# PolyChord/PolyChordLite

Measured on AMD Instinct MI355X. Metric: likelihood evals/sec, 20D Gaussian nlive=2000, higher is better.
Workload: dtype f64; 1 GPU; configs[1]: 20-D Gaussian, nlive=2000, num_repeats=40, one full run per step; batch_chains=1000, parallelism=repeat-sharded x1, mode=one run at a time per GPU; R runs in step: roofline.in_step

## Files before the change

### polychordlite_amd/csrc/pc_engine.hip

```cpp
#include "pc_state.h"
#include "pc_resume.h"
#include "pc_prior_table.h"
#include "pc_launch.h"
#include "pc_plan.h"
#include <cstdio>
#include <cstdlib>
#include <cstring>
#include <cstdarg>
#include <cmath>
#include <vector>
#include <memory>
#include <string>
#include <chrono>
#include <algorithm>
#include <map>
#include <unordered_map>
#include <atomic>
#include <mutex>
#include <thread>
#include <functional>
#include <exception>
#include <ucontext.h>
#include <array>
#include <sys/mman.h>
// ... 140 lines not shown
    {
        int dev = 0; (void)hipGetDevice(&dev);
        {
            std::lock_guard<std::mutex> g(m);
            for (size_t i = events.size(); i-- > 0;)
                if (events[i].first == dev) { hipEvent_t e = events[i].second; events.erase(events.begin() + i); return e; }
        }
        hipEvent_t e; HIPCHK(hipEventCreate(&e)); return e;
    }
    void put_event(hipEvent_t e) { int dev = 0; (void)hipGetDevice(&dev); std::lock_guard<std::mutex> g(m); events.push_back({dev, e}); }
    std::vector<std::pair<int, hipEvent_t>> sync_events;
    hipEvent_t get_sync_event()
    {
        int dev = 0; (void)hipGetDevice(&dev);
        {
            std::lock_guard<std::mutex> g(m);
            for (size_t i = sync_events.size(); i-- > 0;)
                if (sync_events[i].first == dev) { hipEvent_t e = sync_events[i].second; sync_events.erase(sync_events.begin() + i); return e; }
        }
        hipEvent_t e; HIPCHK(hipEventCreateWithFlags(&e, hipEventDisableTiming)); return e;
    }
    void put_sync_event(hipEvent_t e) { int dev = 0; (void)hipGetDevice(&dev); std::lock_guard<std::mutex> g(m); sync_events.push_back({dev, e}); }
};
HandlePool &hpool() { static HandlePool *p = new HandlePool; return *p; }

#define PC_COPY_N 96
#define PC_COPY_PIECE 4096u
struct PcCopyBatch { const void *src[PC_COPY_N]; void *dst[PC_COPY_N]; unsigned bytes[PC_COPY_N]; };
__global__ __launch_bounds__(256) void k_copy_batch(PcCopyBatch b)
{
    const int i = blockIdx.x;
    const unsigned n = b.bytes[i];
    const char *s = (const char *)b.src[i]; char *d = (char *)b.dst[i];
    if ((((uintptr_t)s | (uintptr_t)d) & 7u) == 0u) {
        const unsigned n8 = n >> 3;
        for (unsigned k = threadIdx.x; k < n8; k += 256) ((unsigned long long *)d)[k] = ((const unsigned long long *)s)[k];
        for (unsigned k = (n8 << 3) + threadIdx.x; k < n; k += 256) d[k] = s[k];
    } else for (unsigned k = threadIdx.x; k < n; k += 256) d[k] = s[k];
}
static void pc_copy_many(const std::vector<std::array<uintptr_t, 3>> &reqs, hipStream_t q)
{
    PcCopyBatch b; int n = 0;
    auto go = [&] { if (n) { hipLaunchKernelGGL(k_copy_batch, dim3(n), dim3(256), 0, q, b); n = 0; } };
    for (const auto &r : reqs) {
        size_t left = r[2]; uintptr_t d = r[0], s = r[1];
        while (left) {
            const unsigned c = (unsigned)std::min<size_t>(left, PC_COPY_PIECE);
            b.dst[n] = (void *)d; b.src[n] = (const void *)s; b.bytes[n] = c; ++n;
            d += c; s += c; left -= c;
            if (n == PC_COPY_N) go();
        }
    }
    go();
}

__global__ void k_engine_spin(long long ticks) { const long long t0 = wall_clock64(); while (wall_clock64() - t0 < ticks) {} }
static bool streams_overlap_test(hipStream_t a, hipStream_t b)
{
    auto both = [&] {
        (void)hipStreamSynchronize(a); (void)hipStreamSynchronize(b);
        const auto t0 = std::chrono::steady_clock::now();
        hipLaunchKernelGGL(k_engine_spin, dim3(1), dim3(64), 0, a, 10000LL);
        hipLaunchKernelGGL(k_engine_spin, dim3(1), dim3(64), 0, b, 10000LL);
        (void)hipStreamSynchronize(a); (void)hipStreamSynchronize(b);
        return std::chrono::duration<double>(std::chrono::steady_clock::now() - t0).count();
    };
    static std::atomic<bool> warmed{false};
    if (!warmed.exchange(true)) (void)both();
    const double two = std::min(both(), both());
    if (pc_env().debug == 5) std::fprintf(stderr, "polychord_hip dbg streams %p %p: both %.1f us\n", (void *)a, (void *)b, two * 1e6);
    return two < 170e-6;
}
struct StreamClasses {
    std::mutex mm;
    std::map<void *, int> cls;
    std::vector<hipStream_t> reps;
    int known(hipStream_t x) { std::lock_guard<std::mutex> g(mm); auto it = cls.find((void *)x); return it == cls.end() ? -1 : it->second; }
    int classify(hipStream_t x)
    {
        std::lock_guard<std::mutex> g(mm);
        auto it = cls.find((void *)x);
        if (it != cls.end()) return it->second;
        int c = -1;
        for (size_t r = 0; r < reps.size() && c < 0; ++r) if (!streams_overlap_test(reps[r], x)) c = (int)r;
        if (c < 0) { c = (int)reps.size(); reps.push_back(x); }
        cls[(void *)x] = c;
        return c;
    }
};
static StreamClasses &sclasses() { static StreamClasses *p = new StreamClasses; return *p; }
static hipStream_t stream_avoiding(std::vector<int> avoid, bool known_only = false);
static hipStream_t stream_beside(std::initializer_list<hipStream_t> others, bool known_only = false)
{
    if (pc_env().side_pick_off) return hpool().get_stream();
    std::vector<int> avoid;
    for (hipStream_t o : others) if (o) { const int c = known_only ? sclasses().known(o) : sclasses().classify(o); if (c >= 0) avoid.push_back(c); }
    return stream_avoiding(avoid, known_only);
}
static hipStream_t stream_avoiding(std::vector<int> avoid, bool known_only)
{
    auto fits = [&](int c) { return c >= 0 && std::find(avoid.begin(), avoid.end(), c) == avoid.end(); };
    if (hipStream_t k = hpool().take_stream_if([&](hipStream_t x) { return fits(sclasses().known(x)); })) return k;
    if (known_only) {
        if (hipStream_t k = hpool().take_stream_if([&](hipStream_t x) { return sclasses().known(x) >= 0; })) return k;
        return hpool().get_stream();
    }
// ... 1289 lines not shown
    {
        const int nprior = cfg.nprior <= 0 ? cfg.nlive : cfg.nprior, nT = S.nT;
        double *rows = dalloc<double>((size_t)nprior * nT), *rl = dalloc<double>(nprior);
        std::vector<double> keep_rows; keep_rows.reserve((size_t)nprior * nT);
        std::vector<double> hrows, hl(nprior);
        int have = 0, attempt0 = 0, last_attempt = -1;
        long long nlike = 0;
        bool direct = true;
        while (have < nprior) {
            pc_count(path, launch_traits());
            if (pc_launch_generate_live(&S, attempt0, nprior, rows, rl, st)) {
                if (pc_rtc_wanted(&S) && pc_rtc_error()) engine_fail(PC_RC_SETTINGS, "%.480s", pc_rtc_error());
                engine_fail(PC_RC_NDIMS, "nDims > 256 unsupported");
            }
            HIPCHK(hipMemcpyAsync(hl.data(), rl, sizeof(double) * nprior, hipMemcpyDeviceToHost, st));
            HIPCHK(hipStreamSynchronize(st));
            int nvalid = 0;
            for (int i = 0; i < nprior; ++i) nvalid += hl[i] > cfg.logzero;
            if (nvalid == nprior && have == 0) { have = nprior; nlike = nprior; last_attempt = nprior - 1; break; }
            direct = false;
            hrows.resize((size_t)nprior * nT);
            HIPCHK(hipMemcpy(hrows.data(), rows, sizeof(double) * (size_t)nprior * nT, hipMemcpyDeviceToHost));
            for (int i = 0; i < nprior && have < nprior; ++i)
                if (hl[i] > cfg.logzero) { keep_rows.insert(keep_rows.end(), hrows.begin() + (size_t)i * nT, hrows.begin() + (size_t)(i + 1) * nT); have++; nlike++; last_attempt = attempt0 + i; }
                else ndiscarded++;
            attempt0 += nprior;
        }
        if (!direct) HIPCHK(hipMemcpy(rows, keep_rows.data(), sizeof(double) * (size_t)nprior * nT, hipMemcpyHostToDevice));
        pc_launch_install_live(&S, rows, nprior, st);
        h_ctl->nlike = nlike; h_ctl->nlike_device = nlike;
        HIPCHK(hipMemcpyAsync(&S.ctl->nlike, &h_ctl->nlike, sizeof(long long), hipMemcpyHostToDevice, st));
        HIPCHK(hipStreamSynchronize(st));
        if (S.seq_mode) {
            int a = last_attempt + 1;
            for (; S.ngrade <= 1; ++a) {
                double l1 = 0.0;
                pc_count(path, launch_traits());
                (void)pc_launch_generate_live(&S, a, 1, rows, rl, st);
                HIPCHK(hipMemcpyAsync(&l1, rl, sizeof(double), hipMemcpyDeviceToHost, st));
                HIPCHK(hipStreamSynchronize(st));
                if (l1 > cfg.logzero) break;
            }
            h_ctl->seq = (unsigned long long)(a + (S.ngrade <= 1 ? 1 : 0)) * S.D;
            HIPCHK(hipMemcpy(&S.ctl->seq, &h_ctl->seq, sizeof(unsigned long long), hipMemcpyHostToDevice));
        }
        dfree(rows); dfree(rl);
        call_dumper(2);
        if (nprior > cfg.nlive) {
            pc_count(path, PcTrimLive{}); pc_launch_consume(&S, 2, 0, st);
            read_ctl();
        }
    }

    void stream_dead()
    {
        const size_t nd = (size_t)h_ctl->ndead;
        if (!h_dead || nd > h_dead_cap || nd <= h_dead_copied) return;
        if (ev_apply) HIPCHK(hipStreamWaitEvent(st_copy, ev_apply, 0));
        HIPCHK(hipMemcpyAsync(h_dead + h_dead_copied * S.nT, S.dead + h_dead_copied * S.nT,
                              sizeof(double) * (nd - h_dead_copied) * S.nT, hipMemcpyDeviceToHost, st_copy));
        h_dead_copied = nd;
    }

    void export_resume(PcResume &r)
    {
        HIPCHK(hipStreamSynchronize(st));
        const int D = S.D, nT = S.nT, nc = h_ctl->ncluster, ncd = std::min(h_ctl->ncluster_dead, S.maxc_dead), maxc = S.maxc;
        r = PcResume{};
        r.nDims = D; r.nDerived = S.nDer; r.ndead = h_ctl->ndead; r.ncluster = nc; r.ncluster_dead = ncd;
        {
            long ng[PC_MAX_GRADE];
            grade_counts(ng);
            r.grade_dims.clear(); r.num_repeats.clear(); r.nlike.clear();
            for (int g = 0; g < S.ngrade; ++g) {
                r.grade_dims.push_back((g + 1 < S.ngrade ? S.g_off[g + 1] : D) - S.g_off[g]);
                r.num_repeats.push_back(S.g_nr[g]); r.nlike.push_back(ng[g]);
            }
        }
        r.logZ = h_ctl->logZ; r.logZ2 = h_ctl->logZ2; r.logX_last_update = h_ctl->logX_last_update;
        r.thin_posterior = cfg.boost_posterior < 0.0 ? 1.0 : cfg.boost_posterior / (double)S.nr;
        auto take = [&](const double *p) { auto v = dl(p, std::max(1, nc)); v.resize(nc); return v; };
        r.logLp = take(S.logLp); r.logXp = take(S.logXp); r.logZXp = take(S.logZXp); r.logZp = take(S.logZp);
        r.logZp2 = take(S.logZp2); r.logZpXp = take(S.logZpXp);
        auto xq = dl(S.XpXq, (size_t)maxc * maxc);
        r.logXpXq.assign((size_t)nc * nc, 0.0);
        for (int q = 0; q < nc; ++q) for (int p = 0; p < nc; ++p) r.logXpXq[(size_t)q * nc + p] = xq[(size_t)p * maxc + q];
        r.logZp_dead = dl(S.logZp_dead, std::max(1, ncd)); r.logZp_dead.resize(ncd);
        r.logZp2_dead = dl(S.logZp2_dead, std::max(1, ncd)); r.logZp2_dead.resize(ncd);
        auto cov = dl(S.cov, (size_t)std::max(1, nc) * D * D), ch = dl(S.chol, (size_t)std::max(1, nc) * D * D);
        r.covmat.assign((size_t)nc * D * D, 0.0); r.cholesky.assign((size_t)nc * D * D, 0.0);
        for (int c = 0; c < nc; ++c) for (int j = 0; j < D; ++j) for (int a = 0; a < D; ++a) {
            r.covmat[((size_t)c * D + j) * D + a] = cov[((size_t)c * D + a) * D + j];
            r.cholesky[((size_t)c * D + j) * D + a] = ch[((size_t)c * D + a) * D + j];
        }
        auto cn = dl(S.cl_n, std::max(1, nc)); auto cl = dl(S.cl_list, (size_t)maxc * S.Ncap);
        auto rows = dl(S.live, (size_t)S.Ncap * nT); auto uid = dl(S.cl_uid, std::max(1, nc));
        r.nlive.assign(nc, 0); r.imin.assign(nc, 1); r.live.assign(nc, {}); r.nphantom.assign(nc, 0); r.phantom.assign(nc, {});
        for (int c = 0; c < nc; ++c) {
            r.nlive[c] = cn[c];
            double lo = PC_HUGE;
            for (int k = 0; k < cn[c]; ++k) {
                const double *row = rows.data() + (size_t)cl[(size_t)c * S.Ncap + k] * nT;
                r.live[c].insert(r.live[c].end(), row, row + nT);
                if (row[S.l0] < lo) { lo = row[S.l0]; r.imin[c] = k + 1; }
            }
        }
        const int nph = h_ctl->nphantom;
        auto ph = dl(S.phantom, (size_t)std::max(1, nph) * nT); auto pc = dl(S.ph_cuid, std::max(1, nph));
        for (int j = 0; j < nph; ++j)
            for (int c = 0; c < nc; ++c)
                if (uid[c] == pc[j]) { r.phantom[c].insert(r.phantom[c].end(), ph.begin() + (size_t)j * nT, ph.begin() + (size_t)(j + 1) * nT); r.nphantom[c]++; break; }
        r.dead = dl(S.dead, (size_t)std::max(1, r.ndead) * nT); r.dead.resize((size_t)r.ndead * nT);
        r.logweights = dl(S.dead_logw, std::max(1, r.ndead)); r.logweights.resize(r.ndead);
// ... 90 lines not shown
        put(S.logZp, r.logZp); put(S.logZXp, r.logZXp); put(S.logZp2, r.logZp2); put(S.logZpXp, r.logZpXp);
        { std::vector<double> t(maxc, 0.0); std::copy(r.logXp.begin(), r.logXp.end(), t.begin()); ul(S.logXp, t); }
        std::vector<double> xq((size_t)maxc * maxc, 0.0);
        for (int q = 0; q < nc; ++q) for (int p = 0; p < nc; ++p) xq[(size_t)p * maxc + q] = r.logXpXq[(size_t)q * nc + p];
        ul(S.XpXq, xq);
        std::vector<double> cov((size_t)maxc * D * D, 0.0), ch((size_t)maxc * D * D, 0.0);
        for (int c = 0; c < maxc; ++c) for (int a = 0; a < D; ++a) { cov[((size_t)c * D + a) * D + a] = 1.0; ch[((size_t)c * D + a) * D + a] = 1.0; }
        for (int c = 0; c < nc; ++c) for (int j = 0; j < D; ++j) for (int a = 0; a < D; ++a) {
            cov[((size_t)c * D + a) * D + j] = r.covmat[((size_t)c * D + j) * D + a];
            ch[((size_t)c * D + a) * D + j] = r.cholesky[((size_t)c * D + j) * D + a];
        }
        ul(S.cov, cov); ul(S.chol, ch);
        const int ncd = std::min(r.ncluster_dead, S.maxc_dead);
        { std::vector<double> a(r.logZp_dead.begin(), r.logZp_dead.begin() + ncd), b(r.logZp2_dead.begin(), r.logZp2_dead.begin() + ncd); ul(S.logZp_dead, a); ul(S.logZp2_dead, b); }
        if (sc.ok) ul(S.cl_uid_dead, sc.uid_dead);
        std::vector<double> ph((size_t)std::max(1, nph) * nT), phL(std::max(1, nph));
        std::vector<unsigned> phC(std::max(1, nph)); std::vector<unsigned long long> phU(std::max(1, nph));
        int j = 0;
        for (int c = 0; c < nc; ++c)
            for (int k = 0; k < r.nphantom[c]; ++k, ++j) {
                std::memcpy(ph.data() + (size_t)j * nT, r.phantom[c].data() + (size_t)k * nT, sizeof(double) * nT);
                phL[j] = ph[(size_t)j * nT + S.l0]; phC[j] = uid[c]; phU[j] = 0xFFFFFFFF00000000ull | (unsigned)j;
            }
        if (nph) { ul(S.phantom, ph); ul(S.ph_logL, phL); ul(S.ph_cuid, phC); ul(S.ph_uid, phU); }
        if (r.ndead) {
            ul(S.dead, r.dead); ul(S.dead_logw, r.logweights);
            std::vector<double> z(r.ndead, 0.0), en(r.ndead);
            for (int i = 0; i < r.ndead; ++i) en[i] = r.dead[(size_t)i * nT + S.b0];
            ul(S.dead_postX, z); ul(S.dead_postZ, z); ul(S.dead_entry, en);
            std::vector<unsigned> du(r.ndead, 0u);
            if (sc.ok) du = sc.dead_cuid;
            ul(S.dead_cuid, du);
        }
        PcCtl c0 = *h_ctl;
        c0.status = nc >= 1 ? PC_ST_RUNNING : PC_ST_DONE; c0.ncluster = nc; c0.ncluster_dead = ncd; c0.ndead = r.ndead; c0.nphantom = nph;
        c0.logZ = r.logZ; c0.logZ2 = r.logZ2; c0.logX_last_update = r.logX_last_update; c0.next_cluster_uid = sc.ok ? sc.next_uid : (unsigned)nc + 1;
        c0.nlike = 0;
        for (size_t g = 0; g < r.nlike.size(); ++g) { c0.nlike += r.nlike[g]; if (g >= 1 && g < PC_MAX_GRADE) nlike_g[g] = r.nlike[g]; }
        c0.nlike_device = c0.nlike; c0.i_nursery = 0; c0.failures = 0;
        HIPCHK(hipMemcpy(S.ctl, &c0, sizeof(PcCtl), hipMemcpyHostToDevice));
        *h_ctl = c0;
        return true;
    }

    struct ActiveRun {
        int d; std::atomic<int> *flag;
        ActiveRun(int dv, std::atomic<int> *f) : d(dv & 63), flag(f) { g_active_runs.fetch_add(1); g_active_dev[d].fetch_add(1); std::lock_guard<std::mutex> g(g_run_mutex); g_run_stop.push_back(flag); }
        ~ActiveRun() { g_active_runs.fetch_sub(1); g_active_dev[d].fetch_sub(1); std::lock_guard<std::mutex> g(g_run_mutex); g_run_stop.erase(std::find(g_run_stop.begin(), g_run_stop.end(), flag)); }
    };
    std::unique_ptr<ActiveRun> active_run;
    using clk = std::chrono::steady_clock;
    clk::time_point r_t0, r_t1, r_t2;
    unsigned r_batch = 0; bool r_sort_valid = false, r_fresh = false; int r_nursery_left = 0;
    PcRunPlan plan{};
    int r_rc = 0;

    int run(pchip_result *out)
    {
        int rc = begin();
        if (rc >= 0) return rc;
        while (true) {
            if (!round_enqueue()) break;
            while (!round_ready()) __builtin_ia32_pause();
            if (!round_finish()) break;
        }
        if (r_rc != 0) return r_rc;
        return end(out);
    }

    int begin()
    {
        active_run.reset(new ActiveRun(dev, &stop));
        r_t0 = clk::now();
        h_dead_cap = (size_t)S.Dcap; h_dead = halloc<double>(h_dead_cap * S.nT); h_dead_copied = 0;
        bool resumed = false;
        if (cfg.resume_read) {
            if (FILE *probe = std::fopen(cfg.resume_read, "r")) {
                std::fclose(probe);
                PcResume rs; std::string err;
                if (!pc_resume_read(cfg.resume_read, rs, err) || !import_resume(rs, err)) { std::fprintf(stderr, "polychord_hip: %s\n", err.c_str()); return 6; }
                resumed = true;
                int ntot = 0;
                for (int v : rs.nlive) ntot += v;
                if (ntot > cfg.nlive && rs.ncluster == 1) { pc_count(path, PcTrimLive{}); pc_launch_consume(&S, 2, 0, st); read_ctl(); ntot = cfg.nlive; }
                resume_static = (ntot == cfg.nlive);
                resume_batch0 = (unsigned)rs.ndead;
            }
        }
        if (!resumed) { if (callback_mode) generate_live_callback(); else generate_live(); }
        if (stop.load(std::memory_order_relaxed)) return 5;
        if (cb_auto_batch && !(cb_eval_seconds >= 0.0 && cb_eval_seconds < 2e-6)) { B = B_small; S.B = B; }
        r_t1 = clk::now();
        r_batch = resume_batch0;
        r_sort_valid = false;
        r_nursery_left = 0;
        make_plan();
        S.defer_update = plan.defer ? 1 : 0; S.pool = plan.pool ? 1 : 0;
        if (S.pool) {
            pool_cursor = h_ctl->nphantom;
            babies_own = S.babies;
            if (g_cap_phantoms.load() <= 0) {
                size_t free_b = 0, total_b = 0;
                (void)hipMemGetInfo(&free_b, &total_b);
                const double need = 2.0 * 2.0 * (double)S.Pcap * ((double)S.nT * 8.0 + 24.0);
                if (need < 0.4 * (double)free_b) grow_phantoms(2LL * S.Pcap);
            }
        }
        r_rc = 0;
        return -1;
    }

    void make_plan()
    {
        const int nprior0 = cfg.nprior <= 0 ? cfg.nlive : cfg.nprior;
        PcRunFacts f{};
        f.ablate = cfg.ablate; f.force_general = cfg.force_general;
        f.fixed_nlive = (cfg.n_nlives == 0) && (nprior0 >= cfg.nlive) && resume_static;
        f.par_fits = pc_par_fits(&S) != 0; f.fast_fits = pc_fast_fits(&S) != 0; f.fused_fits_one = pc_update_fused_ok(&S, 1) != 0;
        f.clustering = cfg.do_clustering != 0; f.boost = cfg.boost_posterior != 0.0;
        f.dumper = dumper != nullptr; f.on_update = on_update != nullptr; f.resume_write = cfg.resume_write != nullptr;
        f.seq_mode = S.seq_mode != 0; f.posteriors = cfg.posteriors || cfg.equals;
        f.callback = callback_mode;
        plan = pc_plan_run(f);
    }
    bool other_active() const { return g_active_dev[dev & 63].load(std::memory_order_relaxed) > 1; }
    bool cohort_general_ok() const
    {
        return !pc_env().cohort_general_off && S.ngrade <= 1 && !S.seq_mode && S.like.kind != PC_LIKE_CORR_GAUSSIAN && S.like.kind != PC_LIKE_CALLBACK && S.prior.kind != PCHIP_PRIOR_TABLE;
    }
    PcNurseryFacts nursery_facts(unsigned batch) const
    {
        PcNurseryFacts f{};
        f.in_step = co != nullptr; f.other_active = other_active(); f.callback = callback_mode; f.D = S.D;
        f.ring = raw_buf[1] != nullptr;
        const RawSlot &rs = ring[batch % raw_depth];
        f.slot_ready = rs.valid && rs.batch == batch && rs.B == B;
        f.second_stream = co && co->st2 && raw_depth >= 2;
        f.splittable = pc_nhats_splittable(&S) != 0; f.fusable = pc_slice_fusable(&S) != 0; f.bases_t = pc_bases_t_ok(&S) != 0;
        f.slice_t = pc_slice_t_ok(&S, h_ctl->ncluster) != 0;
        f.cohort_general = cohort_general_ok();
        f.traits = launch_traits();
        return f;
    }
    bool enqueue_nursery()
    {
        unsigned &batch = r_batch; int &nursery_left = r_nursery_left;
        if (S.pool) {
            if (pool_cursor + (long long)B * S.nr > S.Pcap) pool_compact();
            S.pool_base = (int)pool_cursor; S.pool_rows = B * S.nr; S.babies = S.phantom + (size_t)pool_cursor * S.nT;
            pool_cursor += (long long)B * S.nr;
        }
        {
            hipEvent_t e0 = kt.begin(KT_NHATS);
            const PcNurseryChoice ch = pc_choose_nursery(plan, nursery_facts(batch));
            pc_count(path, ch);
            int bases_seq = 0;
            switch (ch.bases) {
            case PC_BASES_READY: case PC_BASES_PART1: case PC_BASES_PART1_STEP: {
                RawSlot &rs = ring[batch % raw_depth];
                S.nhat_raw = raw_buf[batch % raw_depth];
                if (ch.bases == PC_BASES_READY) { if (!rs.waited) HIPCHK(hipStreamWaitEvent(st, rs.ready, 0)); bases_seq = rs.co_seq; }
                else {
                    if (rs.valid) HIPCHK(hipStreamWaitEvent(st, rs.ready, 0));
                    if (ch.bases == PC_BASES_PART1_STEP) co->rec(rec_bases(S, batch, B));
                    else (void)pc_launch_nhats_part(&S, batch, B, 1, st, ch.packed ? 1 : 0);
                }
                rs.valid = false;
                if (ch.part2) { if (co) { co->flush(); co->wait_next(); } (void)pc_launch_nhats_part(&S, batch, B, 2, st, 0); }
                break;
            }
            case PC_BASES_NHATS_G: co->rec(rec_nhats_g(S, batch, B)); break;
            case PC_BASES_WHOLE:
                if (co) co->flush();
                if (pc_launch_nhats(&S, batch, B, st)) { std::fprintf(stderr, "polychord_hip: nDims unsupported\n"); r_rc = 3; return false; }
                break;
            }
            kt.end(KT_NHATS, e0);
            hipEvent_t e1 = kt.begin(KT_SLICE);
            switch (ch.sampler) {
            case PC_SAMPLER_CALLBACK:
                if (co) co->flush();
                slice_callback(batch);
                if (stop.load(std::memory_order_relaxed)) { r_rc = 5; return false; }
                break;
            case PC_SAMPLER_LANE: (void)stage(rec_slice(S, batch, B, bases_seq)); break;
            case PC_SAMPLER_WAVE_STEP: co->rec(rec_slice_g(S, batch, B, ch.fused, ch.fused ? bases_seq : 0)); break;
            case PC_SAMPLER_WAVE:
                if (co) { co->flush(); co->wait_next(); }
                if (ch.fused ? pc_launch_slice_fused(&S, batch, B, st) : pc_launch_slice(&S, batch, B, st)) {
                    if (pc_rtc_wanted(&S) && pc_rtc_error()) { std::fprintf(stderr, "polychord_hip: %s\n", pc_rtc_error()); r_rc = 1; return false; }
                    std::fprintf(stderr, "polychord_hip: nDims unsupported\n"); r_rc = 3; return false;
                }
                break;
            }
            if (ch.ahead == PC_AHEAD_STEP) bases_ahead(batch);
            kt.end(KT_SLICE, e1);
            if (ch.ahead == PC_AHEAD_SIDE) side_prefetch(batch);
            if (S.ngrade > 1) HIPCHK(hipMemcpyAsync(h_nlike_g.data(), S.ch_nlike_g, sizeof(int) * h_nlike_g.size(), hipMemcpyDeviceToHost, st));
            batch++; tm.batches++;
            S.nn_valid = 0; nursery_left = B;
        }
        return true;
    }

    void bases_ahead(unsigned cur)
    {
        const unsigned x = cur + 1;
        RawSlot &rn = ring[x % raw_depth];
        if (rn.valid && rn.batch == x && rn.B == B) return;
        PcState S1 = S; S1.nhat_raw = raw_buf[x % raw_depth];
        co->rec(rec_bases_next(S1, x, B));
        rn.valid = true; rn.batch = x; rn.B = B; rn.waited = true; rn.co_seq = co->seq_for_next();
    }

    void ensure_side()
    {
        if (st_side) return;
        st_side = stream_beside({st, st_copy}); ev_main = hpool().get_sync_event();
        for (int r = 0; r < raw_depth; ++r) { ring[r].ready = hpool().get_sync_event(); ring[r].consumed = hpool().get_sync_event(); }
    }
    hipEvent_t ev_presort_a = nullptr, ev_presort_b = nullptr;
    bool presorted = false;
    void presort_live()
    {
        presorted = false;
        if (pc_env().presort_off || co || other_active() || callback_mode || S.seq_mode || !S.nn_list || h_ctl->ncluster < 2) return;
        ensure_side();
        if (!ev_presort_a) { ev_presort_a = hpool().get_sync_event(); ev_presort_b = hpool().get_sync_event(); }
        HIPCHK(hipEventRecord(ev_presort_a, st)); HIPCHK(hipStreamWaitEvent(st_side, ev_presort_a, 0));
        if (pc_launch_sort_live(&S, st_side) != 0) return;
        HIPCHK(hipEventRecord(ev_presort_b, st_side));
        presorted = true;
    }
    void side_prefetch(unsigned cur)
    {
        const unsigned batch = cur;
        {
        ensure_side();
        const bool side_free = pc_env().side_free || (S.D > 64 && !pc_env().side_ordered);
        RawSlot &cur = ring[batch % raw_depth];
        if (side_free) { HIPCHK(hipEventRecord(cur.consumed, st)); cur.used = true; }
        if (!side_free) { HIPCHK(hipEventRecord(ev_main, st)); HIPCHK(hipStreamWaitEvent(st_side, ev_main, 0)); }
        const unsigned xmax = batch + (unsigned)raw_depth - (side_free ? 0u : 1u);
        for (unsigned x = batch + 1; x <= xmax; ++x) {
            RawSlot &rs = ring[x % raw_depth];
            if (rs.valid && rs.batch == x && rs.B == B) continue;
            if (rs.valid) continue;
            if (rs.used) HIPCHK(hipStreamWaitEvent(st_side, rs.consumed, 0));
            PcState S1 = S; S1.nhat_raw = raw_buf[x % raw_depth];
            hipEvent_t es = kt.begin_on(KT_SIDE, st_side);
            (void)pc_launch_nhats_part(&S1, x, B, 1, st_side, (cfg.ablate & PC_ABL_BASES_PACKED) ? 1 : 0);
            kt.end_on(KT_SIDE, es, st_side);
            HIPCHK(hipEventRecord(rs.ready, st_side));
            rs.valid = true; rs.batch = x; rs.B = B; rs.waited = false;
        }
    }
    }

    PcContractFacts contract_facts(int nursery_left) const
    {
        PcContractFacts f{};
        f.ncluster = h_ctl->ncluster; f.nursery_left = nursery_left;
        f.in_step = co != nullptr; f.cohort_general = cohort_general_ok();
        f.nn_lists = S.nn_list && !pc_env().nn_lists_off; f.nn_valid = S.nn_valid != 0;
        f.cl_fits = f.ncluster > 1 && pc_consume_cl_fits(&S, f.ncluster) != 0;
        f.clp_fits = f.cl_fits && pc_consume_clp_fits(&S, f.ncluster) != 0;
        return f;
    }
    bool round_enqueue()
    {
        unsigned &batch = r_batch; bool &sort_valid = r_sort_valid; int &nursery_left = r_nursery_left;
        {
            if (h_ctl->status == PC_ST_DONE) return false;
            if (h_ctl->status == PC_ST_ERROR) { std::fprintf(stderr, "polychord_hip: device error %d\n", h_ctl->error); r_rc = 2; return false; }
            bool fresh_nursery = false;
            if (h_ctl->i_nursery == 0) {
                fresh_nursery = true;
                DbgSpan dbg_t{g_dbg_nursery_ns};
                if (plan.cl_ok) presort_live();
                if (!enqueue_nursery()) return false;
            }
            if (fresh_nursery) { DbgSpan dbg_t{g_dbg_capacity_ns}; ensure_capacity(); }
            hipEvent_t e2 = kt.begin(KT_CONSUME);
            int rc2 = 0;
            const PcContractChoice ch = pc_choose_contract(plan, contract_facts(nursery_left));
            pc_count(path, ch);
            launch_stamp();
            if (presorted && (co || !(h_ctl->ncluster > 1))) { HIPCHK(hipStreamWaitEvent(st, ev_presort_b, 0)); presorted = false; }
            switch (ch.kind) {
            case PC_CONTRACT_PAR:
                S.nn_valid = 0;
                if (!sort_valid) { rc2 = stage(rec_sort(S)); sort_valid = true; }
                rc2 = rc2 || stage(rec_consume(S));
                break;
            case PC_CONTRACT_FAST:
                if (co) co->flush();
                sort_valid = false; S.nn_valid = 0;
                rc2 = pc_launch_consume_fast(&S, 0, st); pc_launch_ph_prepare(&S, st);
                break;
            case PC_CONTRACT_CL_STEP:
                sort_valid = false;
                if (ch.want_nn) { co->rec(rec_nn(S, nursery_left)); S.nn_valid = 1; }
                co->rec(rec_sort(S));
                co->rec(rec_consume_cl(S, h_ctl->ncluster > 64));
                break;
            case PC_CONTRACT_CL: case PC_CONTRACT_GENERAL: {
                sort_valid = false;
                if (co) co->flush();
                bool sorted_now = false;
                if (presorted) { HIPCHK(hipStreamWaitEvent(st, ev_presort_b, 0)); sorted_now = fresh_nursery; presorted = false; }
                if (ch.want_nn) {
                    if (!sorted_now) sorted_now = pc_launch_sort_live(&S, st) == 0;
                    pc_launch_nn_lists(&S, nursery_left, sorted_now ? 1 : 0, st);
                    S.nn_valid = 1;
                }
                if (ch.kind == PC_CONTRACT_CL) rc2 = (sorted_now ? 0 : pc_launch_sort_live(&S, st)) || pc_launch_consume_cl(&S, h_ctl->ncluster, st);
                else rc2 = pc_launch_consume(&S, 0, (h_ctl->ncluster > 1) ? 1 : 0, st);
                break;
            }
            }
            if (rc2) { std::fprintf(stderr, "polychord_hip: nlive too large for the LDS-resident contraction\n"); r_rc = 4; return false; }
            kt.end(KT_CONSUME, e2);
            hipEvent_t e3 = kt.begin(KT_APPLY);
            (void)stage(rec_apply(S, batch - 1, B));
            kt.end(KT_APPLY, e3);
            if (st_side) { RawSlot &rs = ring[batch % raw_depth]; if (rs.valid && rs.batch == batch && !rs.waited) { HIPCHK(hipStreamWaitEvent(st, rs.ready, 0)); rs.waited = true; } }
            r_fresh = fresh_nursery;
            ready_spins = 0;
        }
        return true;
    }

    bool finish_may_wait() const
    {
        const bool upd = h_ctl->status == PC_ST_UPDATE || (h_ctl->upd_pending && h_ctl->status == PC_ST_RUNNING);
        return upd && pc_choose_update(plan, update_facts(1)).may_wait;
    }
    bool round_finish()
    {
        unsigned &batch = r_batch; int &nursery_left = r_nursery_left; const bool fresh_nursery = r_fresh;
        (void)batch;
        {
            if (fresh_nursery && h_ctl->status == PC_ST_DONE && h_ctl->i_nursery == B) tm.batches--;
            nursery_left = h_ctl->i_nursery;
            tally_grades();
            tm.rounds++;
            if (h_ctl->status == PC_ST_UPDATE || (h_ctl->upd_pending && h_ctl->status == PC_ST_RUNNING)) {
                do_update(h_ctl->status != PC_ST_UPDATE); h_ctl->status = PC_ST_RUNNING; h_ctl->upd_pending = 0;
                if ((size_t)h_ctl->ndead >= h_dead_copied + 4 * (size_t)cfg.nlive) {
                if (!ev_apply) ev_apply = hpool().get_sync_event();
                HIPCHK(hipEventRecord(ev_apply, st));
                stream_dead();
                }
            }
        }
        return true;
    }

    struct EndState {
        double *hlive = nullptr; int *hcl = nullptr; double *d_pmax = nullptr, *h_part = nullptr, *h_zp = nullptr;
        int nc_end = 0, ncd_max = 0, pmD = 0, pm_nb = 0, pm_pw = 0; clk::time_point t2;
    } es;
    hipStream_t st_fin = nullptr; hipEvent_t ev_fin = nullptr;
    void end_a(bool fused_final = false)
    {
        if (co && !fused_final) co->flush();
        bool &sort_valid = r_sort_valid;
        es.t2 = clk::now();
        st_fin = st;
        if (co && fused_final && !pc_env().cohort_final_aside_off && st_copy && st_copy != st && h_ctl->ncluster > 1) {
            ev_fin = hpool().get_sync_event();
            HIPCHK(hipEventRecord(ev_fin, st));
            HIPCHK(hipStreamWaitEvent(st_copy, ev_fin, 0));
            st_fin = st_copy;
        }
        hipStream_t st = st_fin;
        const int nT = S.nT;
        es.hlive = halloc<double>((size_t)S.Ncap * nT); es.hcl = halloc<int>(S.Ncap);
        HIPCHK(hipMemcpyAsync(es.hlive, S.live, sizeof(double) * (size_t)S.Ncap * nT, hipMemcpyDeviceToHost, st));
        HIPCHK(hipMemcpyAsync(es.hcl, S.live_cluster, sizeof(int) * S.Ncap, hipMemcpyDeviceToHost, st));
        es.nc_end = h_ctl->ncluster;
        if (h_ctl->ncluster == 0) {
        } else if (plan.par_ok && h_ctl->ncluster == 1) {
            path[PCHIP_PATH_KILLOFF_PAR]++;
            if (co && sort_valid) { co->rec(rec_final(S)); if (!fused_final) co->flush(); }
            else {
            if (!sort_valid) (void)pc_launch_sort_live(&S, st);
            (void)pc_launch_final_par(&S, st);
            }
        } else if (h_ctl->ncluster > 1 && pc_launch_killoff_cl(&S, h_ctl->ncluster, st) == 0) {
            path[PCHIP_PATH_KILLOFF_CL]++;
        } else if (plan.fast_ok && h_ctl->ncluster == 1 && pc_launch_consume_fast(&S, 1, st) == 0) path[PCHIP_PATH_KILLOFF_FAST]++;
        else { path[PCHIP_PATH_KILLOFF_GENERAL]++; pc_launch_consume(&S, 1, (h_ctl->ncluster > 1 && !S.seq_mode) ? 1 : 0, st); }
        if (!fused_final) end_a2();
    }
    void end_a2()
    {
        hipStream_t st = st_fin ? st_fin : this->st;
        es.pmD = S.D + S.nDer; es.pm_nb = pc_post_blocks(); es.pm_pw = 3 * es.pmD + 1;
        es.ncd_max = std::min(h_ctl->ncluster_dead + h_ctl->ncluster, S.maxc_dead);
        es.d_pmax = dalloc<double>(2 * (size_t)es.pm_nb); es.h_part = halloc<double>((size_t)es.pm_nb * es.pm_pw);
        es.h_zp = halloc<double>(2 * (size_t)std::max(1, es.ncd_max));
        pc_launch_post_moments(&S, -1, es.d_pmax, es.h_part, st);
        if (es.ncd_max > 0) {
            HIPCHK(hipMemcpyAsync(es.h_zp, S.logZp_dead, sizeof(double) * es.ncd_max, hipMemcpyDeviceToHost, st));
            HIPCHK(hipMemcpyAsync(es.h_zp + es.ncd_max, S.logZp2_dead, sizeof(double) * es.ncd_max, hipMemcpyDeviceToHost, st));
        }
        HIPCHK(hipMemcpyAsync(h_ctl, S.ctl, sizeof(PcCtl), hipMemcpyDeviceToHost, st));
        if (ev_fin) HIPCHK(hipEventRecord(ev_fin, st));
    }
    void end_wait_aside() { if (ev_fin) { HIPCHK(hipEventSynchronize(ev_fin)); hpool().put_sync_event(ev_fin); ev_fin = nullptr; } }
    int end(pchip_result *out) { end_a(); HIPCHK(hipStreamSynchronize(st)); end_wait_aside(); return end_b(out); }
    int end_b(pchip_result *out)
    {
        struct HostBuf { EndState &e; ~HostBuf() { if (e.hlive) hfree(e.hlive); if (e.hcl) hfree(e.hcl); e.hlive = nullptr; e.hcl = nullptr; } } hb{es};
        double *hlive = es.hlive; int *hcl = es.hcl; double *d_pmax = es.d_pmax, *h_part = es.h_part, *h_zp = es.h_zp;
        const int nc_end = es.nc_end, ncd_max = es.ncd_max, pmD = es.pmD, pm_nb = es.pm_nb, pm_pw = es.pm_pw, nT = S.nT;
        const auto t0 = r_t0, t1 = r_t1; auto t2 = es.t2;
        HIPCHK(hipGetLastError());
        nph_stale = false;
        kt.collect();
        if (cfg.boost_posterior != 0.0 && (cfg.posteriors || cfg.equals) && h_ctl->nphantom > 0) {
            pc_launch_clean(&S, h_ctl->nphantom, keep, blk, d_total, ph2, phL2, phC2, phU2, nullptr, st);
            collect_phantom_posteriors(h_ctl->nphantom);
        }
        call_dumper(1);
        write_resume();
        auto t3 = clk::now();
        tm.t_gen = std::chrono::duration<double>(t1 - t0).count();
        tm.t_loop = std::chrono::duration<double>(t2 - t1).count();
        tm.t_final = std::chrono::duration<double>(t3 - t2).count();
        tm.t_total = std::chrono::duration<double>(t3 - t0).count();
        std::memset(out, 0, sizeof(*out));
        out->logZ = std::max(-PC_HUGE, 2 * h_ctl->logZ - 0.5 * h_ctl->logZ2);
        out->varlogZ = h_ctl->logZ2 - 2 * h_ctl->logZ;
        out->ndead = h_ctl->ndead; out->nlike = h_ctl->nlike; out->niter = h_ctl->niter;
        out->nlike_failed = h_ctl->nlike_failed; out->ncluster_peak = ncluster_peak; out->epoch_discard = S.epoch_discard;
        path[PCHIP_PATH_NN_FALLBACKS] = (long)h_ctl->nn_fallbacks; path[PCHIP_PATH_POOL_MODE] = S.pool; path[PCHIP_PATH_DEFER_UPDATE] = S.defer_update;
        for (int k = 0; k < PCHIP_PATH_COUNT; ++k) out->path[k] = path[k];
        grade_counts(out->nlike_grade);
        out->ncluster = nc_end; out->ncluster_dead = h_ctl->ncluster_dead; out->nbatches = tm.batches;
        out->nrounds = tm.rounds; out->nupdates = tm.updates; out->nTotal = nT; out->batch = B;
        out->t_generate = tm.t_gen; out->t_loop = tm.t_loop; out->t_final = tm.t_final; out->t_total = tm.t_total;
        for (int k = 0; k < KT_N; ++k) { out->k_time_s[k] = kt.total_ms[k] * 1e-3; out->k_launches[k] = kt.launches[k]; }
        const int dbg_lvl = pc_env().debug;
        if (dbg_lvl >= 3) std::fprintf(stderr, "polychord_hip dbg general: term %lld identify %lld kill+add %lld tail %lld cycles; %lld chains identified from the candidate lists, %lld of them fell back to the full search\n", h_ctl->gen_cyc[0], h_ctl->gen_cyc[1], h_ctl->gen_cyc[2], h_ctl->gen_cyc[3], h_ctl->nn_walks, h_ctl->nn_fallbacks);
        if (dbg_lvl == 4) std::fprintf(stderr, "polychord_hip dbg par: stage+search %lld rank-sort %lld accept %lld merge+slots %lld evidence %lld triggers %lld publish %lld cycles\n", h_ctl->dbg[0], h_ctl->dbg[1], h_ctl->dbg[2], h_ctl->dbg[3], h_ctl->dbg[4], h_ctl->dbg[5], h_ctl->dbg[6]);
        if (dbg_lvl == 4) std::fprintf(stderr, "polychord_hip dbg par: %lld evidence scans as pairs (terms beyond one scale)\n", h_ctl->dbg[7]);
        if (dbg_lvl == 4 && h_ctl->wave_cyc[0]) std::fprintf(stderr, "polychord_hip dbg clp (several clusters; the line above then reads: decisions | order of deaths + slots | counts + volumes | volume sum + step 0's phantoms | prefix sums + commit | waves 1-3 | write back | passes): wave 1 %lld wave 2 %lld wave 3 %lld phantom wave %lld cycles\n", h_ctl->wave_cyc[0], h_ctl->wave_cyc[1], h_ctl->wave_cyc[2], h_ctl->wave_cyc[3]);
        if (dbg_lvl == 2) std::fprintf(stderr, "polychord_hip dbg: loop cycles %lld passB %lld (%lld flushes) accept-steps %lld (%lld) ins-rescan %lld (%lld) reject-steps cycles %lld\n", h_ctl->dbg[0], h_ctl->dbg[1], h_ctl->dbg[4], h_ctl->dbg[2], h_ctl->dbg[3], h_ctl->dbg[5], h_ctl->dbg[6], h_ctl->dbg[7]);
        if ((size_t)h_ctl->ndead > h_dead_cap) {
            HIPCHK(hipStreamSynchronize(st_copy));
            hfree(h_dead); h_dead_cap = (size_t)h_ctl->ndead; h_dead = halloc<double>(h_dead_cap * nT); h_dead_copied = 0;
        }
        stream_dead();
        out->dead = h_dead; h_dead = nullptr;
        out->logweights = halloc<double>(std::max(1, h_ctl->ndead));
        HIPCHK(hipMemcpyAsync(out->logweights, S.dead_logw, sizeof(double) * h_ctl->ndead, hipMemcpyDeviceToHost, st_copy));
        out->entry = halloc<double>(std::max(1, h_ctl->ndead));
        HIPCHK(hipMemcpyAsync(out->entry, S.dead_entry, sizeof(double) * h_ctl->ndead, hipMemcpyDeviceToHost, st_copy));
        int nl = 0;
        for (int s = 0; s < S.Ncap; ++s) nl += hcl[s] >= 0;
        out->nlive_final = nl;
        out->live = (double *)std::malloc(sizeof(double) * (size_t)std::max(1, nl) * nT);
        out->live_cluster = (int *)std::malloc(sizeof(int) * (size_t)std::max(1, nl));
        for (int s = 0, k = 0; s < S.Ncap; ++s) if (hcl[s] >= 0) { std::memcpy(out->live + (size_t)k * nT, hlive + (size_t)s * nT, sizeof(double) * nT); out->live_cluster[k] = hcl[s]; k++; }
        const int ncd = std::min(h_ctl->ncluster_dead, S.maxc_dead);
        out->nZp = ncd;
        out->logZp = (double *)std::malloc(sizeof(double) * std::max(1, ncd));
        out->varlogZp = (double *)std::malloc(sizeof(double) * std::max(1, ncd));
        if (ncd > ncd_max) engine_fail(PC_RC_DEVICE, "more retired clusters (%d) than the final stage could have left (%d)", ncd, ncd_max);
        for (int i = 0; i < ncd; ++i) { const double zp = h_zp[i], zp2 = h_zp[ncd_max + i]; out->logZp[i] = 2 * zp - 0.5 * zp2; out->varlogZp[i] = zp2 - 2 * zp; }
        hfree(h_zp);
        const int D = pmD, nb = pm_nb, pw = pm_pw;
        out->post_mean = (double *)std::calloc(D, sizeof(double)); out->post_var = (double *)std::calloc(D, sizeof(double));
        double sw = 0.0;
        for (int b = 0; b < nb; ++b) {
            sw += h_part[(size_t)b * pw + 2 * D];
            for (int d = 0; d < D; ++d) { out->post_mean[d] += h_part[(size_t)b * pw + d]; out->post_var[d] += h_part[(size_t)b * pw + D + d]; }
        }
        for (int d = 0; d < D; ++d) {
            const double dm = out->post_mean[d] / sw;
            out->post_mean[d] = h_part[2 * D + 1 + d] + dm;
            out->post_var[d] = std::max(0.0, out->post_var[d] / sw - dm * dm);
        }
        dfree(d_pmax); hfree(h_part);
        long long *h_nrec = nullptr;
        if (cfg.device_records && h_ctl->ndead > 0) {
            const long long cap = h_ctl->ndead;
            double *blk_rec = (double *)pc_cache_dev_alloc(pc_records_block_bytes(cap, nT));
            if (!blk_rec) engine_fail(PC_RC_MEMORY, "no device memory for the run's records (%lld rows)", cap);
            h_nrec = halloc<long long>(1);
            if (pc_pack_lived_device(S.dead, S.dead_logw, S.dead_entry, cap, nT, cfg.logzero, blk_rec, cap, h_nrec, st_copy) != 0) { pc_cache_dev_free(blk_rec); hfree(h_nrec); engine_fail(PC_RC_DEVICE, "packing the run's records"); }
            out->d_records = blk_rec; out->records_cap = (long)cap; out->records_device = dev;
        }
        HIPCHK(hipStreamSynchronize(st_copy));
        if (h_nrec) { out->n_records = (long)*h_nrec; hfree(h_nrec); }
        active_run.reset();
        return 0;
    }

    void destroy(bool streams_idle = false)
    {
        active_run.reset();
        if (!streams_idle) {
        if (st) (void)hipStreamSynchronize(st);
        if (st_copy) (void)hipStreamSynchronize(st_copy);
        if (st_side) (void)hipStreamSynchronize(st_side);
// ... 509 lines not shown
```

### polychordlite_amd/csrc/pc_plan.h

```cpp
#pragma once
#include "pc_state.h"
#include "polychord_hip.h"
#include <cstdlib>
#include <algorithm>

struct PcEnv {
    static bool set(const char *n) { return std::getenv(n) != nullptr; }
    static bool zero(const char *n) { const char *e = std::getenv(n); return e && std::atoi(e) == 0; }
    static int num(const char *n, int dflt) { const char *e = std::getenv(n); return e ? std::atoi(e) : dflt; }
    const int debug = num("PC_DEBUG", 0);
    const bool poison = set("PC_POISON");
    const bool side_pick_off = set("PC_SIDE_PICK_OFF");
    const bool ms_pre_off = set("PC_MS_PRE_OFF");
    const bool nhats_split_off = set("PC_NHATS_SPLIT_OFF");
    const int raw_depth = std::max(2, num("PC_RAW_DEPTH", 3));
    const bool copy_batch_off = set("PC_COPY_BATCH_OFF");
    const bool notify_off = set("PC_NOTIFY_OFF");
    const bool cluster_batch_off = set("PC_CLUSTER_BATCH_OFF");
    const bool presort_off = set("PC_PRESORT_OFF");
    const bool side_free = set("PC_SIDE_FREE"), side_ordered = set("PC_SIDE_ORDERED");
    const bool nn_lists_off = set("PC_NN_LISTS_OFF");
    const bool cohort_general_off = zero("PC_COHORT_GENERAL");
    const bool cohort_final_aside_off = zero("PC_COHORT_FINAL_ASIDE");
    const bool cohort_side_off = zero("PC_COHORT_SIDE");
    const bool cohort_copy_streams_off = zero("PC_COHORT_COPY_STREAMS");
    const bool cohort_fibers_off = zero("PC_COHORT_FIBERS");
    const int cohort_setup_threads = std::max(1, num("PC_COHORT_SETUP_THREADS", 1));
};
inline const PcEnv &pc_env() { static const PcEnv e; return e; }

struct PcRunFacts {
    int ablate, force_general;
    bool fixed_nlive;
    bool par_fits, fast_fits;
    bool fused_fits_one;
    bool clustering, boost;
    bool dumper, on_update, resume_write;
    bool seq_mode, posteriors;
    bool callback;
};
enum PcCtlRead { PC_CTL_NONE = 0,
                 PC_CTL_EARLY,
                 PC_CTL_LATE };
struct PcRunPlan {
    int ablate; bool seq_mode;
    bool static_ok, par_ok, fast_ok;
    bool cl_ok;
    bool fused_update;
    bool host_tied;
    bool sees_update;
    bool sees_update_seq;
    bool sees_update_fused;
    PcCtlRead ctl;
    bool hook_late;
    bool defer;
    bool pool;
};
inline PcRunPlan pc_plan_run(const PcRunFacts &f)
{
    PcRunPlan p{};
    p.ablate = f.ablate; p.seq_mode = f.seq_mode;
    p.static_ok = f.fixed_nlive && f.force_general != 1;
    p.fast_ok = p.static_ok && f.fast_fits;
    p.par_ok = p.static_ok && f.force_general == 0 && f.par_fits;
    p.cl_ok = p.static_ok && f.force_general == 0 && !(f.ablate & PC_ABL_CONSUME_GENERAL);
    p.fused_update = !f.clustering && !f.boost && !(f.ablate & PC_ABL_NO_FUSED_UPDATE);
    const bool seq_post = f.seq_mode && f.posteriors;
    p.host_tied = f.dumper || f.on_update || f.resume_write;
    p.sees_update = p.host_tied || f.clustering || f.boost || seq_post;
    p.sees_update_seq = p.host_tied || f.clustering || f.boost || f.seq_mode;
    p.sees_update_fused = p.host_tied || seq_post;
    p.ctl = !p.sees_update ? PC_CTL_NONE : (f.clustering && !(p.host_tied || f.boost || seq_post)) ? PC_CTL_LATE : PC_CTL_EARLY;
    p.hook_late = f.boost && f.posteriors;
    p.defer = !(f.ablate & PC_ABL_NO_DEFER) && p.par_ok && !p.sees_update_seq && p.fused_update && f.fused_fits_one;
// ... 63 lines not shown

struct PcContractFacts {
    int ncluster, nursery_left;
    bool in_step, cohort_general;
    bool nn_lists;
    bool nn_valid;
    bool cl_fits, clp_fits;
};
enum PcContract { PC_CONTRACT_PAR = 0,
                  PC_CONTRACT_FAST,
                  PC_CONTRACT_CL_STEP,
                  PC_CONTRACT_CL,
                  PC_CONTRACT_GENERAL };
struct PcContractChoice {
    PcContract kind;
    bool want_nn;
    bool clp;
};
inline PcContractChoice pc_choose_contract(const PcRunPlan &p, const PcContractFacts &f)
{
    PcContractChoice c{};
    if (p.par_ok && f.ncluster == 1) { c.kind = PC_CONTRACT_PAR; return c; }
    if (p.fast_ok && f.ncluster == 1) { c.kind = PC_CONTRACT_FAST; return c; }
    c.want_nn = f.ncluster > 1 && f.nn_lists && !f.nn_valid && !p.seq_mode && f.nursery_left > 1;
    const bool use_cl = p.cl_ok && (f.nn_valid || c.want_nn) && !p.seq_mode && f.ncluster > 1 && f.cl_fits;
    c.kind = !use_cl ? PC_CONTRACT_GENERAL : (f.in_step && f.cohort_general) ? PC_CONTRACT_CL_STEP : PC_CONTRACT_CL;
    c.clp = use_cl && f.clp_fits;
    return c;
}

struct PcUpdateFacts {
    bool rows;
    bool fused_fits;
    int ncluster;
};
enum PcUpdate { PC_UPDATE_FUSED = 0,
                PC_UPDATE_STEPS };
struct PcUpdateChoice {
    PcUpdate kind;
    bool need_count;
    PcCtlRead ctl; bool hook_late;
    bool may_wait;
};
inline PcUpdateChoice pc_choose_update(const PcRunPlan &p, const PcUpdateFacts &f)
{
    PcUpdateChoice c{};
    c.kind = (p.fused_update && f.rows && f.fused_fits) ? PC_UPDATE_FUSED : PC_UPDATE_STEPS;
    c.need_count = c.kind == PC_UPDATE_FUSED ? p.sees_update_fused : p.sees_update;
    c.ctl = p.ctl; c.hook_late = p.hook_late;
    c.may_wait = p.sees_update_seq || f.ncluster > 1 || !f.fused_fits;
    return c;
}

inline void pc_count(long *path, const PcLaunchTraits &t)
{
    if (t.rtc) path[PCHIP_PATH_SOURCE_KERNELS]++;
    if (t.src_terms) path[PCHIP_PATH_SOURCE_TERMS]++;
    if (t.device_prior) path[PCHIP_PATH_DEVICE_PRIOR]++;
}
inline void pc_count(long *path, const PcNurseryChoice &c)
{
    switch (c.sampler) {
    case PC_SAMPLER_CALLBACK: break;
    case PC_SAMPLER_LANE: path[PCHIP_PATH_SLICE_LANE]++; break;
    case PC_SAMPLER_WAVE_STEP: path[PCHIP_PATH_SLICE_WAVE]++; pc_count(path, PcLaunchTraits{c.traits.rtc, false, false}); break;
    case PC_SAMPLER_WAVE: path[PCHIP_PATH_SLICE_WAVE]++; pc_count(path, c.traits); break;
    }
}
inline void pc_count(long *path, const PcContractChoice &c)
{
    if (c.want_nn) path[PCHIP_PATH_NN_LISTS]++;
    switch (c.kind) {
    case PC_CONTRACT_PAR: path[PCHIP_PATH_CONSUME_PAR]++; break;
    case PC_CONTRACT_FAST: path[PCHIP_PATH_CONSUME_FAST]++; break;
    case PC_CONTRACT_CL_STEP: case PC_CONTRACT_CL: path[c.clp ? PCHIP_PATH_CONSUME_CL : PCHIP_PATH_CONSUME_CL_SERIAL]++; break;
    case PC_CONTRACT_GENERAL: path[PCHIP_PATH_CONSUME_GENERAL]++; break;
    }
}
inline void pc_count(long *path, const PcUpdateChoice &c) { path[c.kind == PC_UPDATE_FUSED ? PCHIP_PATH_UPDATE_FUSED : PCHIP_PATH_UPDATE_STEPS]++; }
struct PcTrimLive {};
inline void pc_count(long *path, const PcTrimLive &) { path[PCHIP_PATH_CONSUME_GENERAL]++; }
```

### polychordlite_amd/csrc/pc_state.h

```cpp
#pragma once
#include "pc_dev.h"

enum { PC_ST_RUNNING = 0, PC_ST_DONE = 1, PC_ST_UPDATE = 2, PC_ST_ERROR = 4 };
enum { PC_ERR_NONE = 0, PC_ERR_PHANTOM_CAP = 1, PC_ERR_DEAD_CAP = 2, PC_ERR_CLUSTER_CAP = 3, PC_ERR_NOSLOT = 4 };

enum { PC_ABL_FUNCTOR = 1 << 0, PC_ABL_NO_POOL = 1 << 1, PC_ABL_NO_DEFER = 1 << 2, PC_ABL_NO_FUSED_UPDATE = 1 << 3, PC_ABL_PAIR_SCANS = 1 << 4,
       PC_ABL_CONSUME_GENERAL = 1 << 5, PC_ABL_SLICE_LANE = 1 << 6, PC_ABL_BASES_PACKED = 1 << 7, PC_ABL_CL_END_AT_DEATH = 1 << 8,
       PC_ABL_KILLOFF_GENERAL = 1 << 9, PC_ABL_CONSUME_CL_SERIAL = 1 << 10, PC_ABL_RETIRED_11 = 1 << 11, PC_ABL_RETIRED_12 = 1 << 12,
       PC_ABL_NO_HELPER = 1 << 13, PC_ABL_QC_BY_CHAIN = 1 << 14, PC_ABL_RTC_BUILTINS = 1 << 15, PC_ABL_UPDATE_CHAIN = 1 << 16, PC_ABL_TRACE_CHOL = 1 << 30 };

#define PC_MASK_WORDS 16

struct PcCtl {
    int status;
    int error;
    int i_nursery;
    int admin_epoch;
    int failures;
    int ncluster;
    int ncluster_dead;
    int ndead;
    int nphantom;
    int seg_hi, seg_lo;
    int cluster_deleted;
    unsigned batch_id;
    unsigned next_cluster_uid;
    long long nlike;
    long long niter;
    long long nlike_device;
    long long nlike_failed;
    double logZ, logZ2;
    double logX_last_update;
    double live_logZ;
    unsigned long long seq;
    long long dbg[8];
    long long gen_cyc[4];
    long long nn_walks, nn_fallbacks;
    int upd_pending, upd_marks;
    int upd_tmark;
    int upd_T, upd_ts;
    int upd_nph0;
    int upd_keep_thr, upd_pad;
    double upd_thr;
    int chol_suspect, chol_pad;
    long long wave_cyc[4];
};

#define PC_MAX_GRADE 8
#define PC_NN_K 8
#define PC_NN_NONE (-2147483647 - 1)
#define PC_CUID_NONE 0xFFFFFFFEu

struct alignas(16) PcPlanHead {
    int dead_idx;
    int dead_src;
    int ph_base;
    unsigned dead_cuid;
    unsigned ph_cuid;
    int ph_count;
    double logw;
    double postX, postZ;
    double postXs;
// ... 190 lines not shown
```

Before: 1.321 billion likelihood evals/s.

## Export dead points with a small copy kernel queued behind the slice event

Adds a k_export_dead kernel that copies dead-point rows from device memory straight into the host buffer with a few workgroups, as an alternative to hipMemcpyAsync. A policy function picks between kernel and memcpy and decides when the export is issued: behind the slice event, at apply time, or gathered on updates. The aim is to overlap the dead-point download with the slice stage and avoid DMA setup stalls. The kernel path is only chosen when the run is not in-step and no other run is active, so it costs some compute units and adds timing complexity, with env-var variants kept for experimentation.

```diff
diff --git a/polychordlite_amd/csrc/pc_engine.hip b/polychordlite_amd/csrc/pc_engine.hip
--- a/polychordlite_amd/csrc/pc_engine.hip
+++ b/polychordlite_amd/csrc/pc_engine.hip
@@ -216,6 +216,18 @@
         }
     }
     go();
+}
+
+#define PC_EXPORT_WG 4
+__global__ __launch_bounds__(256) void k_export_dead(const unsigned long long *__restrict__ src, unsigned long long *__restrict__ dst, size_t n)
+{
+    const size_t stride = (size_t)PC_EXPORT_WG * 256;
+    size_t k = (size_t)blockIdx.x * 256 + threadIdx.x;
+    for (; k + 3 * stride < n; k += 4 * stride) {
+        const unsigned long long a = src[k], b = src[k + stride], c = src[k + 2 * stride], d = src[k + 3 * stride];
+        dst[k] = a; dst[k + stride] = b; dst[k + 2 * stride] = c; dst[k + 3 * stride] = d;
+    }
+    for (; k < n; k += stride) dst[k] = src[k];
 }
 
 __global__ void k_engine_spin(long long ticks) { const long long t0 = wall_clock64(); while (wall_clock64() - t0 < ticks) {} }
@@ -1611,13 +1623,15 @@
         }
     }
 
-    void stream_dead()
+    PcExportFacts export_facts() const { PcExportFacts f{}; f.in_step = co != nullptr; f.other_active = other_active(); f.slice_event = r_slice_event; return f; }
+    void stream_dead(const PcExportChoice &ex, hipEvent_t behind)
     {
         const size_t nd = (size_t)h_ctl->ndead;
         if (!h_dead || nd > h_dead_cap || nd <= h_dead_copied) return;
-        if (ev_apply) HIPCHK(hipStreamWaitEvent(st_copy, ev_apply, 0));
-        HIPCHK(hipMemcpyAsync(h_dead + h_dead_copied * S.nT, S.dead + h_dead_copied * S.nT,
-                              sizeof(double) * (nd - h_dead_copied) * S.nT, hipMemcpyDeviceToHost, st_copy));
+        if (behind) HIPCHK(hipStreamWaitEvent(st_copy, behind, 0));
+        const size_t off = h_dead_copied * S.nT, n = (nd - h_dead_copied) * S.nT;
+        if (ex.kernel) hipLaunchKernelGGL(k_export_dead, dim3(PC_EXPORT_WG), dim3(256), 0, st_copy, (const unsigned long long *)(S.dead + off), (unsigned long long *)(h_dead + off), n);
+        else HIPCHK(hipMemcpyAsync(h_dead + off, S.dead + off, sizeof(double) * n, hipMemcpyDeviceToHost, st_copy));
         h_dead_copied = nd;
     }
 
@@ -1814,6 +1828,8 @@
     using clk = std::chrono::steady_clock;
     clk::time_point r_t0, r_t1, r_t2;
     unsigned r_batch = 0; bool r_sort_valid = false, r_fresh = false; int r_nursery_left = 0;
+    bool export_pending = false;
+    bool r_slice_event = false;
     PcRunPlan plan{};
     int r_rc = 0;
 
@@ -1856,6 +1872,7 @@
         r_batch = resume_batch0;
         r_sort_valid = false;
         r_nursery_left = 0;
+        r_slice_event = false;
         make_plan();
         S.defer_update = plan.defer ? 1 : 0; S.pool = plan.pool ? 1 : 0;
         if (S.pool) {
@@ -1957,6 +1974,7 @@
             }
             if (ch.ahead == PC_AHEAD_STEP) bases_ahead(batch);
             kt.end(KT_SLICE, e1);
+            r_slice_event = false;
             if (ch.ahead == PC_AHEAD_SIDE) side_prefetch(batch);
             if (S.ngrade > 1) HIPCHK(hipMemcpyAsync(h_nlike_g.data(), S.ch_nlike_g, sizeof(int) * h_nlike_g.size(), hipMemcpyDeviceToHost, st));
             batch++; tm.batches++;
@@ -2002,7 +2020,12 @@
         const bool side_free = pc_env().side_free || (S.D > 64 && !pc_env().side_ordered);
         RawSlot &cur = ring[batch % raw_depth];
         if (side_free) { HIPCHK(hipEventRecord(cur.consumed, st)); cur.used = true; }
-        if (!side_free) { HIPCHK(hipEventRecord(ev_main, st)); HIPCHK(hipStreamWaitEvent(st_side, ev_main, 0)); }
+        if (!side_free) {
+            HIPCHK(hipEventRecord(ev_main, st)); HIPCHK(hipStreamWaitEvent(st_side, ev_main, 0));
+            r_slice_event = true;
+            const PcExportChoice ex = pc_choose_export(plan, export_facts());
+            if (ex.behind_slice) { if (pc_env().export_variant == 2 || pc_env().export_variant == 4) export_pending = true; else stream_dead(ex, ev_main); }
+        }
         const unsigned xmax = batch + (unsigned)raw_depth - (side_free ? 0u : 1u);
         for (unsigned x = batch + 1; x <= xmax; ++x) {
             RawSlot &rs = ring[x % raw_depth];
@@ -2087,6 +2110,7 @@
             (void)stage(rec_apply(S, batch - 1, B));
             kt.end(KT_APPLY, e3);
             if (st_side) { RawSlot &rs = ring[batch % raw_depth]; if (rs.valid && rs.batch == batch && !rs.waited) { HIPCHK(hipStreamWaitEvent(st, rs.ready, 0)); rs.waited = true; } }
+            if (export_pending) { export_pending = false; stream_dead(pc_choose_export(plan, export_facts()), ev_main); }
             r_fresh = fresh_nursery;
             ready_spins = 0;
         }
@@ -2107,13 +2131,14 @@
             nursery_left = h_ctl->i_nursery;
             tally_grades();
             tm.rounds++;
-            if (h_ctl->status == PC_ST_UPDATE || (h_ctl->upd_pending && h_ctl->status == PC_ST_RUNNING)) {
-                do_update(h_ctl->status != PC_ST_UPDATE); h_ctl->status = PC_ST_RUNNING; h_ctl->upd_pending = 0;
-                if ((size_t)h_ctl->ndead >= h_dead_copied + 4 * (size_t)cfg.nlive) {
+            const bool upd = h_ctl->status == PC_ST_UPDATE || (h_ctl->upd_pending && h_ctl->status == PC_ST_RUNNING);
+            if (upd) { do_update(h_ctl->status != PC_ST_UPDATE); h_ctl->status = PC_ST_RUNNING; h_ctl->upd_pending = 0; }
+            const PcExportChoice ex = pc_choose_export(plan, export_facts());
+            const size_t gather = ex.every_round ? 1 : 4 * (size_t)cfg.nlive;
+            if (!ex.behind_slice && (upd || ex.every_round) && (size_t)h_ctl->ndead >= h_dead_copied + gather) {
                 if (!ev_apply) ev_apply = hpool().get_sync_event();
                 HIPCHK(hipEventRecord(ev_apply, st));
-                stream_dead();
-                }
+                stream_dead(ex, ev_apply);
             }
         }
         return true;
@@ -2215,7 +2240,7 @@
             HIPCHK(hipStreamSynchronize(st_copy));
             hfree(h_dead); h_dead_cap = (size_t)h_ctl->ndead; h_dead = halloc<double>(h_dead_cap * nT); h_dead_copied = 0;
         }
-        stream_dead();
+        { PcExportChoice exf = pc_choose_export(plan, export_facts()); if (pc_env().export_variant >= 3) exf.kernel = false; stream_dead(exf, nullptr); }
         out->dead = h_dead; h_dead = nullptr;
         out->logweights = halloc<double>(std::max(1, h_ctl->ndead));
         HIPCHK(hipMemcpyAsync(out->logweights, S.dead_logw, sizeof(double) * h_ctl->ndead, hipMemcpyDeviceToHost, st_copy));
diff --git a/polychordlite_amd/csrc/pc_plan.h b/polychordlite_amd/csrc/pc_plan.h
--- a/polychordlite_amd/csrc/pc_plan.h
+++ b/polychordlite_amd/csrc/pc_plan.h
@@ -20,6 +20,8 @@
     const bool presort_off = set("PC_PRESORT_OFF");
     const bool side_free = set("PC_SIDE_FREE"), side_ordered = set("PC_SIDE_ORDERED");
     const bool nn_lists_off = set("PC_NN_LISTS_OFF");
+    const bool export_at_apply = set("PC_EXPORT_AT_APPLY");
+    const int export_variant = num("PC_EXPORT_VARIANT", 0);
     const bool cohort_general_off = zero("PC_COHORT_GENERAL");
     const bool cohort_final_aside_off = zero("PC_COHORT_FINAL_ASIDE");
     const bool cohort_side_off = zero("PC_COHORT_SIDE");
@@ -189,6 +191,26 @@
     return c;
 }
 
+struct PcExportFacts {
+    bool in_step, other_active;
+    bool slice_event;
+};
+struct PcExportChoice {
+    bool kernel;
+    bool behind_slice;
+    bool every_round;
+};
+inline PcExportChoice pc_choose_export(const PcRunPlan &p, const PcExportFacts &f)
+{
+    PcExportChoice c{};
+    c.kernel = !f.in_step && !f.other_active && !(p.ablate & PC_ABL_DEAD_MEMCPY);
+    const int v = pc_env().export_variant;
+    const bool gather = v == 1 || v == 3;
+    c.every_round = c.kernel && f.slice_event && pc_env().export_at_apply && !gather;
+    c.behind_slice = c.kernel && f.slice_event && !c.every_round && !gather;
+    return c;
+}
+
 inline void pc_count(long *path, const PcLaunchTraits &t)
 {
     if (t.rtc) path[PCHIP_PATH_SOURCE_KERNELS]++;
diff --git a/polychordlite_amd/csrc/pc_state.h b/polychordlite_amd/csrc/pc_state.h
--- a/polychordlite_amd/csrc/pc_state.h
+++ b/polychordlite_amd/csrc/pc_state.h
@@ -7,7 +7,8 @@
 enum { PC_ABL_FUNCTOR = 1 << 0, PC_ABL_NO_POOL = 1 << 1, PC_ABL_NO_DEFER = 1 << 2, PC_ABL_NO_FUSED_UPDATE = 1 << 3, PC_ABL_PAIR_SCANS = 1 << 4,
        PC_ABL_CONSUME_GENERAL = 1 << 5, PC_ABL_SLICE_LANE = 1 << 6, PC_ABL_BASES_PACKED = 1 << 7, PC_ABL_CL_END_AT_DEATH = 1 << 8,
        PC_ABL_KILLOFF_GENERAL = 1 << 9, PC_ABL_CONSUME_CL_SERIAL = 1 << 10, PC_ABL_RETIRED_11 = 1 << 11, PC_ABL_RETIRED_12 = 1 << 12,
-       PC_ABL_NO_HELPER = 1 << 13, PC_ABL_QC_BY_CHAIN = 1 << 14, PC_ABL_RTC_BUILTINS = 1 << 15, PC_ABL_UPDATE_CHAIN = 1 << 16, PC_ABL_TRACE_CHOL = 1 << 30 };
+       PC_ABL_NO_HELPER = 1 << 13, PC_ABL_QC_BY_CHAIN = 1 << 14, PC_ABL_RTC_BUILTINS = 1 << 15, PC_ABL_UPDATE_CHAIN = 1 << 16,
+       PC_ABL_DEAD_MEMCPY = 1 << 17, PC_ABL_TRACE_CHOL = 1 << 30 };
 
 #define PC_MASK_WORDS 16
 
```

Measured after the change: 1.228 billion likelihood evals/s. 0.929x the previous value.
